# songweige/rich-text-to-image

Measured on AMD Instinct MI355X. Metric: denoising steps/sec (SDXL 1024^2, 50-step, 4 regions), higher is better.
Workload: dtype bf16; 1 GPU; SDXL RegionDiffusionXL 1024x1024, R=4 regions, inject_selfattn=0.5, 50-step Euler, CFG 5.0, 7 UNet forwards/step batched, random-init SDXL-base weights; global_batch=1, parallelism=seed-parallel x1 (1 weight broadcast, no per-step collectives), elide_dead_forwards=False

## Files before the change

### include/rtdiff.h

```cpp
#ifndef RTDIFF_H
#define RTDIFF_H
#include <stdint.h>
#ifdef __cplusplus
extern "C" {
#endif

#define RT_OK 0
#define RT_E_INVALID (-1)
#define RT_E_HIP (-2)
#define RT_E_STATE (-3)
#define RT_E_MISSING_WEIGHT (-4)
#define RT_E_UNSUPPORTED (-5)

#define RT_MAX_LEVELS 4
#define RT_MAX_STREAMS 16

enum { RT_DTYPE_F32 = 0, RT_DTYPE_F16 = 1, RT_DTYPE_BF16 = 2 };
enum { RT_SCHED_EULER = 0, RT_SCHED_PNDM = 1, RT_SCHED_DPMPP_1 = 2, RT_SCHED_DPMPP_2 = 3,
       RT_SCHED_EULER_A = 4, RT_SCHED_DPMPP_SDE_1 = 5, RT_SCHED_DPMPP_SDE_2 = 6 };

typedef struct rt_config {
    int n_levels;
    int block_out_channels[RT_MAX_LEVELS];
    int down_has_attn[RT_MAX_LEVELS];
// ... 108 lines not shown
int rt_trace_module_count(rt_engine* e);
int rt_trace_module_info(rt_engine* e, int idx, char* name, int name_cap, int* channels, int* downshift);

int rt_op_gemm(const void* A, const void* W, const float* bias, void* out, const void* res, const float* temb,
               int mode, int epi, int M, int N, int K, int lda, int ldw, int ldo, int ldres, int temb_ld,
               int rows_per_batch, int Hin, int Win, int Cin, int Hout, int Wout, void* stream);
int rt_op_attention(const void* Q, int ldq, const void* K, int ldk, const void* VT, int ldvt, void* O, int ldo,
                    const int* q_src_host, const int* k_src_host, const int* v_src_host, const int* wset_host,
                    const float* wabs, const float* wsgn, int B, int H, int N, int NK, int nk_valid, int DP, int cross,
                    void* stream);
int rt_op_attention_keys(const void* Q, int ldq, const void* K, int ldk, const void* VT, int ldvt, void* O, int ldo,
                         const int* q_src_host, const int* prompt_host, const int* wset_host, const float* wabs, const float* wsgn,
                         const int* key_counts_host, int B, int H, int N, int NK, int DP, void* stream);
int rt_op_ip_attention(const void* Q, int ldq, const void* Kip, int ldk, const void* VTip, int ldvt, void* O, int ldo,
                       const int* slot_host, const int* count_host, const float* scale_host, int B, int H, int N, int DP, void* stream);
int rt_op_identity_attention(const void* VT, int ldvt, void* O, int ldo, const int* entry_host, int n, int B, int H, int N, int DP, void* stream);
int rt_op_pag_fold(float* eps, int n_streams, int h, int w, const int* stream_host, const int* twin_host, const float* ratio_host, int n, void* stream);
int rt_op_lora_add(const void* X, int ldx, const void* down, int ldd, const void* up, int ldu, const float* alpha_over_rank,
                   const int* col_adapter, void* Y, int ldy, int form, const int* row_host, const float* scale_host, int B, int rows, int K,
                   int N, int R, int* launched, void* stream);
int rt_op_attention_units_plan(const int* q_src, const int* k_src, int B, int tokens, int DP, int mode, int* launch_of, int* unit_of, int* members_of);
int rt_op_gemm16_pick(int conv3x3, int epi, int streams, int rows_per_stream, int N, int K_or_Cin, int weights_on_rows, int* w_stationary);
int rt_op_split_plan(int conv3x3, int epi, int streams, int rows_per_stream, int N, int K_or_Cin, int* route, int* slices);
enum { RT_ROUTE_TILE = 0        ,
       RT_ROUTE_G16 = 1         ,
       RT_ROUTE_G16_UP2 = 2     ,
       RT_ROUTE_PATCH = 3       ,
       RT_ROUTE_PATCH_SPLIT = 4 ,
       RT_ROUTE_KSPLIT = 5      ,
       RT_ROUTE_TRIPLE = 6       };
int rt_op_gemm_route(int mode, int epi, int M, int N, int K, int lda, int ldw, int ldo, int rows_per_batch, int Hin, int Win, int Cin,
                     int Hout, int Wout, int* kind, int* variant_or_cfg, int* slices);
int rt_op_gemm16_variant(const void* A, const void* W, const float* bias, void* out, const void* res, int epi, int M, int N, int K, int lda,
                         int ldw, int ldo, int ldres, int weights_on_rows, int variant, int wstat, void* stream);
int rt_op_gemm_pair_pick(int streams_qk, int streams, int rows_per_stream, int Nqk, int Nv, int K);
int rt_op_gemm_qk_vt(const void* X, int ldx, int K, int rows_per_stream, const void* Wqk, const float* bqk, int Mqk, int Nqk, void* qk, int ldqk,
                     const void* Wv, int Nv, int M, void* vt, int ldvt, int* grouped, void* stream);
int rt_op_cross_attn_block(const void* x, const void* wq, const void* wo, const float* bo, const void* kcache, const void* vtcache, int ldvt,
                           const int* prompt_host, const int* wset_host, const float* wabs, const float* wsgn, const void* trunk_in_f16,
                           void* trunk_out_f16, void* q_scratch, void* o_scratch, int B, int N, int C, int H, int DP, void* stream);
int rt_op_groupnorm(const void* x1, const void* x2, int in_type, int C1, int C2, int G, int B, int HW,
                    const float* gamma, const float* beta, float eps, int silu, void* out_bf16, void* raw_out_bf16,
                    void* stream);
int rt_op_groupnorm_form(int in_type, int C1, int C2, int G, int B, int HW);

int rt_op_gemm_hilo(const void* A, const void* A_lo, const void* W, const void* W_lo, const float* bias, float* out_f32, void* pair_lo,
// ... 111 lines not shown
```

### rich-text-to-image_amd/csrc/common.h

```cpp
#pragma once
#include <hip/hip_runtime.h>
#include <stdint.h>
#include <stdio.h>
#include <string>
#include <stdexcept>

typedef uint16_t bf16_t;
typedef __attribute__((ext_vector_type(8))) __bf16 bf16x8;
typedef __attribute__((ext_vector_type(4))) __bf16 bf16x4;
typedef __attribute__((ext_vector_type(16))) float f32x16;
typedef __attribute__((ext_vector_type(4))) float f32x4;

#define RT_OK 0
#define RT_E_INVALID (-1)
#define RT_E_HIP (-2)
#define RT_E_STATE (-3)
#define RT_E_MISSING_WEIGHT (-4)
#define RT_E_UNSUPPORTED (-5)

struct rt_error : std::runtime_error {
    int code;
    rt_error(int c, const std::string& m) : std::runtime_error(m), code(c) {}
};

// ... 105 lines not shown
};
int gemm_ln_emit_bn(const GemmArgs& a);
bool gemm_ln_fold_ok(const GemmArgs& a);
bool gemm16_ln_variant_ok(const GemmArgs& a, int v);
void launch_ln_partials(const f16_t* x, bf16_t* xb, float* part, int rows, int C, int bn, hipStream_t st, int part_ld = 0);
void launch_ln_fold_derive(const bf16_t* W, int ldw, const float* bias, const float* gamma, const float* beta, int N, int K,
                           bf16_t* Wf, float* sc, hipStream_t st);
int gemm16_variant_bn(int v);
bool xattn_fused_supported(int C, int H, int DP, int tokens);
void launch_xattn_fused(const GemmArgs& a, hipStream_t st);
struct XBlockArgs {
    const bf16_t* x; const bf16_t* wq; const bf16_t* wo; const float* bo;
    const bf16_t* kc; const bf16_t* vt;
    const f16_t* res; f16_t* out;
    const float* wabs; const float* wsgn;
    int ldk, ldvt, ldres, ldo;
    int M, tokens, nk_valid, C, H;
    int prompt[RT_MAXB], wset[RT_MAXB];
};
bool xblock_supported(int C, int H, int DP, int tokens);
void launch_xblock(const XBlockArgs& a, hipStream_t st);
void launch_gemm(const GemmArgs& a, hipStream_t st);
struct GemmRoute {
    enum Kind { G16, PATCH, PATCH_SPLIT, KSPLIT, TILE, TRIPLE, G16_UP2 };
    Kind kind = TILE;
    int variant = -1, wstat = 0;
    int slices = 1;
    int cfg = -1;
};
GemmRoute gemm_route(const GemmArgs& a);
bool gemm_pair_output_ok(const GemmArgs& a);
size_t gemm_splitk_scratch_floats(const GemmArgs& a);
void gemm_force_config(int cfg);
enum DebugBit {
    DBG_CONV_IMPLICIT = 0,
    DBG_NO_GEMM16 = 1,
    DBG_NO_SPLIT = 2,
    DBG_CONV_NO_GEMM16 = 3,
    DBG_NO_XATTN_FUSED = 4,
    DBG_STORE_TWO_PASS = 5,
    DBG_STORE_ONE_PASS = 6,
    DBG_TRIPLE = 7,
    DBG_TRIPLE_GEMM16 = 8,
    DBG_TRIPLE_PATCH = 9,
    DBG_CONV3P_NO_TN4 = 10,
    DBG_GN_CHUNK_128 = 11,
    DBG_G16_NO_DEEP = 12,
    DBG_NO_PAIR = 13,
    DBG_ATTN_NO_PRIO = 14,
    DBG_TRIPLE_DENSE = 15,
    DBG_XBLOCK = 16,
    DBG_STORE_OWN_STATS = 17,
    DBG_STORE_APPLY_V1 = 18,
    DBG_NO_CROSS77 = 19,
    DBG_C77_ONE_TILE = 20,
    DBG_C77_TWO_HEADS = 21,
    DBG_NO_LNFOLD = 22,
    DBG_GN_TWO_LAUNCH = 23,
    DBG_ATTN_UNITS = 24,
    DBG_G16_TALL = 27,
    DBG_NO_CHUNK_SPLIT = 28,
    DBG_NO_CHUNK_HALVES = 29,
    DBG_SPLIT_NO_SMALL_ROWS = 30,
};
enum DebugBit2 {
    DBG2_NO_UP2_PHASE = 0,
};
static inline int debug_bit(int flags, int bit) { return (flags >> bit) & 1; }
void gemm_set_debug(int flags);
void gemm_set_debug2(int flags);
bool gemm_lnfold_enabled();
bool gemm_xblock_enabled();
bool gemm_xattn_enabled();
#define RT_G16_NVAR 14
bool gemm16_supported(const GemmArgs& a);
int gemm16_pick(const GemmArgs& a, int weights_on_rows, int* wstat);
void launch_gemm16_variant(const GemmArgs& a, int variant, int wstat, hipStream_t st);
int gemm16_pick_up2(const GemmArgs& a);
void launch_gemm16_up2(const GemmArgs& a, int variant, hipStream_t st);
int gemm16_pair_variant(const GemmArgs& a, int va, int wa, const GemmArgs& b, int vb, int wb);
void launch_gemm16_pair(const GemmArgs& a, const GemmArgs& b, int pair, hipStream_t st);
int gemm_pair_grouped(const GemmArgs& a, const GemmArgs& b);
void launch_gemm_pair(const GemmArgs& a, const GemmArgs& b, hipStream_t st);

struct AttnArgs {
    const bf16_t* Q;  int ldq;
    const bf16_t* K;  int ldk;
    const bf16_t* VT; int ldvt;
    bf16_t* O;        int ldo;
    int q_src[RT_MAXB], k_src[RT_MAXB], v_src[RT_MAXB], wset[RT_MAXB];
    unsigned char ng[RT_MAXB], gvs[RT_MAXB][4], gob[RT_MAXB][4];
    const float* wabs;
    const float* wsgn;
    int B, H, N;
    int NK;
    int nk_valid;
    int nkeys[RT_MAXB];
    int DP;
    int cross;
    int nqb;
    float* stats; int stats_b;
};
// ... 143 lines not shown
```

### rich-text-to-image_amd/csrc/engine.hip

```cpp
#include "common.h"
#include "../../include/rtdiff.h"
#include <map>
#include <mutex>
#include <vector>
#include <string>
#include <cmath>
#include <cstring>
#include <functional>
#include <algorithm>

static thread_local std::string g_create_error;
static thread_local std::string g_op_error;

struct Arena {
    char* base = nullptr;
    size_t off = 0, cap = 0;
    void* alloc(size_t bytes) {
        off = (off + 255) & ~(size_t)255;
        void* p = base ? base + off : (void*)(uintptr_t)(off + 256);
        off += bytes;
        if (base && off > cap) throw rt_error(RT_E_STATE, "arena overflow");
        return p;
    }
};
// ... 2112 lines not shown
                             int epi, int M, int N, int K, int lda, int ldw, int ldo, int ldres, int temb_ld, int rows_per_batch, int Hin,
                             int Win, int Cin, int Hout, int Wout) {
    GemmArgs g{}; g.A = (const bf16_t*)A; g.W = (const bf16_t*)W; g.bias = bias; g.out = out; g.res = res; g.temb = temb;
    g.zero = zero; g.mode = mode; g.epi = epi; g.M = M; g.N = N; g.K = K; g.lda = lda; g.ldw = ldw; g.ldo = ldo;
    g.ldres = ldres; g.temb_ld = temb_ld; g.rows_per_batch = rows_per_batch; g.Hin = Hin; g.Win = Win; g.Cin = Cin;
    g.Hout = Hout; g.Wout = Wout;
    return g;
}
int rt_op_gemm(const void* A, const void* W, const float* bias, void* out, const void* res, const float* temb, int mode,
               int epi, int M, int N, int K, int lda, int ldw, int ldo, int ldres, int temb_ld, int rows_per_batch, int Hin,
               int Win, int Cin, int Hout, int Wout, void* stream) {
    OP_TRY({
        const GemmArgs g = op_gemm_args(A, W, bias, out, res, temb, op_zero_page(), mode, epi, M, N, K, lda, ldw, ldo, ldres, temb_ld, rows_per_batch,
                                        Hin, Win, Cin, Hout, Wout);
        launch_gemm(g, (hipStream_t)stream);
    })
}
static int op_route_kind(const GemmRoute& r, int* v) {
    *v = -1;
    switch (r.kind) {
        case GemmRoute::TILE: *v = r.cfg; return RT_ROUTE_TILE;
        case GemmRoute::G16: *v = r.variant; return RT_ROUTE_G16;
        case GemmRoute::G16_UP2: *v = r.variant; return RT_ROUTE_G16_UP2;
        case GemmRoute::PATCH: return RT_ROUTE_PATCH;
        case GemmRoute::PATCH_SPLIT: return RT_ROUTE_PATCH_SPLIT;
        case GemmRoute::KSPLIT: return RT_ROUTE_KSPLIT;
        case GemmRoute::TRIPLE: return RT_ROUTE_TRIPLE;
    }
    return RT_ROUTE_TILE;
}
int rt_op_gemm_route(int mode, int epi, int M, int N, int K, int lda, int ldw, int ldo, int rows_per_batch, int Hin, int Win, int Cin, int Hout,
                     int Wout, int* kind, int* variant_or_cfg, int* slices) {
    try {
        if (mode < A_DENSE || mode > A_CONV3_S2P0 || epi < EPI_BF16 || epi > EPI_F16 || M <= 0 || N <= 0 || K <= 0) return RT_E_INVALID;
        if (mode != A_DENSE && (rows_per_batch <= 0 || Cin <= 0 || Hin <= 0 || Win <= 0 || Hout <= 0 || Wout <= 0)) return RT_E_INVALID;
        const GemmArgs g = op_gemm_args(nullptr, nullptr, nullptr, nullptr, nullptr, nullptr, nullptr, mode, epi, M, N, K, lda, ldw, ldo, 0, 0,
                                        rows_per_batch, Hin, Win, Cin, Hout, Wout);
        const GemmRoute r = gemm_route(g);
        int v = -1;
        const int k = op_route_kind(r, &v);
        if (kind) *kind = k;
        if (variant_or_cfg) *variant_or_cfg = v;
        if (slices) *slices = r.slices;
        return RT_OK;
    } catch (...) { return RT_E_INVALID; }
}
// ... 129 lines not shown
}
int rt_op_attention_keys(const void* Q, int ldq, const void* K, int ldk, const void* VT, int ldvt, void* O, int ldo, const int* q_src,
                         const int* prompt, const int* wset, const float* wabs, const float* wsgn, const int* key_counts, int B, int H,
                         int N, int NK, int DP, void* stream) {
    OP_TRY({
        RT_REQUIRE(B >= 1 && B <= RT_MAXB && key_counts, "rt_op_attention_keys: batch / key counts");
        RT_REQUIRE(NK == 96 || NK == 192 || NK == 288, "rt_op_attention_keys: NK must be 96, 192 or 288 rows per prompt");
        int p[RT_MAXB], ws[RT_MAXB];
        for (int b = 0; b < B; ++b) {
            RT_REQUIRE(op_key_count_ok(key_counts[b], NK), "rt_op_attention_keys: a key count must be 77 per 96-row chunk of NK");
            p[b] = prompt ? prompt[b] : b; ws[b] = wset ? wset[b] : -1;
        }
        RT_REQUIRE(!q_src, "rt_op_attention_keys: cross launches read Q of their own batch entry (q_src must be NULL)");
        launch_cross(unet_cross_attn_args(AttnIO{(const bf16_t*)Q, ldq, (const bf16_t*)K, ldk, (const bf16_t*)VT, ldvt, (bf16_t*)O, ldo}, p, ws, key_counts, wabs, wsgn,
                                          B, H, N, NK, DP),
                     cross_route(H * DP, H, DP, DP, N, NK, key_counts, B, false, false, false), (hipStream_t)stream);
    })
}
static bool query_args(GemmArgs& g, int mode, int epi, int streams, int rows_per_stream, int N, int K_or_Cin, int weights_on_rows) {
    const int M = streams * rows_per_stream;
    if (mode != A_DENSE) {
        int side = 1; while (side * side < rows_per_stream) ++side;
        if (side * side != rows_per_stream || (mode == A_CONV3_UP2 && side % 2)) return false;
        const int in = mode == A_CONV3_UP2 ? side / 2 : side;
        g = unet_conv3_args(nullptr, nullptr, mode, op_mat(nullptr, nullptr, N, 9 * K_or_Cin), streams, in, in, K_or_Cin, nullptr, epi);
        g.weights_on_rows = weights_on_rows;
    } else if (weights_on_rows) {
        g = unet_vt_args(nullptr, rows_per_stream, op_mat(nullptr, nullptr, N, K_or_Cin), nullptr, K_or_Cin, M, nullptr, M);
        g.epi = epi;
    } else g = unet_dense_args(nullptr, rows_per_stream, nullptr, K_or_Cin, op_mat(nullptr, nullptr, N, K_or_Cin), M, nullptr, N, epi);
    return true;
}
int rt_op_split_plan(int conv3x3, int epi, int streams, int rows_per_stream, int N, int K_or_Cin, int* route, int* slices) {
    try {
        GemmArgs g;
        if (!query_args(g, conv3x3 == 3 ? A_CONV3_UP2 : conv3x3 ? A_CONV3 : A_DENSE, epi, streams, rows_per_stream, N, K_or_Cin, 0)) return RT_E_INVALID;
        const GemmRoute r = gemm_route(g);
        const int kind = r.kind == GemmRoute::KSPLIT ? 1 : r.kind == GemmRoute::PATCH_SPLIT ? 2 : 0;
        if (route) *route = kind;
        if (slices) *slices = kind ? r.slices : 1;
        return RT_OK;
    } catch (...) { return RT_E_INVALID; }
}
int rt_op_gemm16_pick(int conv3x3, int epi, int streams, int rows_per_stream, int N, int K_or_Cin, int weights_on_rows, int* w_stationary) {
    try {
        GemmArgs g;
        if (!query_args(g, conv3x3 ? A_CONV3 : A_DENSE, epi, streams, rows_per_stream, N, K_or_Cin, weights_on_rows)) return -2;
        int ws = 0;
        const int v = gemm16_pick(g, weights_on_rows, &ws);
        if (w_stationary) *w_stationary = ws;
        return v;
    } catch (...) { return -3; }
}
int rt_op_gemm16_variant(const void* A, const void* W, const float* bias, void* out, const void* res, int epi, int M, int N, int K, int lda,
                         int ldw, int ldo, int ldres, int weights_on_rows, int variant, int wstat, void* stream) {
    OP_TRY({
        GemmArgs g = unet_dense_args(op_zero_page(), 0, (const bf16_t*)A, lda, op_mat(W, bias, N, K), M, out, ldo, epi, res, ldres);
        g.ldw = ldw; g.weights_on_rows = weights_on_rows;
        if (variant < 0) { int ws = 0; variant = gemm16_pick(g, weights_on_rows, &ws); wstat = ws; RT_REQUIRE(variant >= 0, "rt_op_gemm16_variant: the family has no tile for this shape"); }
        launch_gemm16_variant(g, variant, wstat, (hipStream_t)stream);
    })
}
int rt_op_gemm_pair_pick(int streams_qk, int streams, int rows_per_stream, int Nqk, int Nv, int K) {
// ... 282 lines not shown
```

### rich-text-to-image_amd/csrc/gemm.hip

```cpp
#include "common.h"
#include <algorithm>
#include <cmath>
#include <map>
#include <tuple>
#include <type_traits>



#define BK 64
#ifndef RT_ABLATE
#define RT_ABLATE 0
#endif

template <int EPI, int TM, int TN, int NWC, int LDS_BYTES, bool PATCH = false>
__device__ __forceinline__ void gemm_epilogue(const GemmArgs& p, f32x16 (&acc)[TM][TN], int wrow0, int wcol0, int lane, int wave_c,
                                              char* smem, int prow_base = 0, int pW = 0) {
    auto grow = [&](int r) { return PATCH ? prow_base + (r >> 4) * pW + (r & 15) : r; };
    constexpr bool F16 = EPI == EPI_F16;
    constexpr bool F32 = EPI == EPI_F32 || F16;
    constexpr int ES = F32 ? 4 : 2;
    constexpr int TO = EPI == EPI_GEGLU ? TN / 2 : TN;
    static_assert(EPI != EPI_GEGLU || TN % 2 == 0, "GEGLU needs value/gate tile pairs in one wave");
    constexpr int MAXROW = LDS_BYTES / NWC / 32;
    constexpr int TS_RAW = (MAXROW - 16) / (32 * ES);
// ... 1050 lines not shown
        case A_CONV3_S2P0 * 8 + EPI_F32: launch_me<A_CONV3_S2P0, EPI_F32>(a, cfg, st); break;
        default: throw rt_error(RT_E_UNSUPPORTED, "gemm: (operand mode, epilogue) combination not built");
    }
    HIP_CHECK(hipGetLastError());
}

static struct GemmSwitches {
    int force_cfg = -1;
    bool conv_patch = true;
    bool use16 = true;
    bool splitk = true;
    bool conv16 = true;
    bool xattn = true;
    bool triple = false, triple16 = false, triple_patch = false, triple_dense = false;
    bool pair = true;
    bool cross77 = true;
    bool xblock = false;
    bool split_small_rows = true;
    bool conv3p_tn4 = true;
    bool chunk_split = true;
    bool chunk_halves = true;
    bool lnfold = true;
    bool up2_phase = true;
} g_sw;
#ifdef RT_PROBE
int g_conv3p_tn = 0;
#endif
void gemm_set_debug(int flags) {
    auto on = [flags](int bit) { return debug_bit(flags, bit); };
    g_sw.conv_patch = !on(DBG_CONV_IMPLICIT); g_sw.use16 = !on(DBG_NO_GEMM16); g_sw.splitk = !on(DBG_NO_SPLIT); g_sw.conv16 = !on(DBG_CONV_NO_GEMM16);
    g_sw.xattn = !on(DBG_NO_XATTN_FUSED); g_sw.xblock = on(DBG_XBLOCK); g_sw.cross77 = !on(DBG_NO_CROSS77); g_sw.pair = !on(DBG_NO_PAIR);
    g_sw.triple = on(DBG_TRIPLE); g_sw.triple16 = on(DBG_TRIPLE_GEMM16); g_sw.triple_patch = on(DBG_TRIPLE_PATCH); g_sw.triple_dense = on(DBG_TRIPLE_DENSE);
    g_sw.split_small_rows = !on(DBG_SPLIT_NO_SMALL_ROWS); g_sw.conv3p_tn4 = !on(DBG_CONV3P_NO_TN4);
    g_sw.chunk_split = !on(DBG_NO_CHUNK_SPLIT); g_sw.chunk_halves = !on(DBG_NO_CHUNK_HALVES); g_sw.lnfold = !on(DBG_NO_LNFOLD);
}
void gemm_set_debug2(int flags) { g_sw.up2_phase = !debug_bit(flags, DBG2_NO_UP2_PHASE); }
void gemm_force_config(int cfg) { g_sw.force_cfg = cfg; }
bool gemm_cross77_enabled() { return g_sw.cross77; }
bool gemm_lnfold_enabled() { return g_sw.lnfold && g_sw.use16 && g_sw.force_cfg < 0; }
bool gemm_xblock_enabled() { return g_sw.xblock && g_sw.use16 && g_sw.force_cfg < 0; }
bool gemm_xattn_enabled() { return g_sw.xattn && g_sw.use16 && g_sw.force_cfg < 0; }

template <int EPI, bool UP2, int TN>
static void launch_conv3p_tn(const GemmArgs& a, int ntm, int slices, hipStream_t st) {
    constexpr int LDS = 2 * (UP2 ? 104 : 328) * 128 + 3 * 32 * TN * 128;
    static bool attr = false;
    if (!attr) {
        HIP_CHECK(hipFuncSetAttribute((const void*)conv3p_kernel<EPI, UP2, TN>, hipFuncAttributeMaxDynamicSharedMemorySize, LDS));
        attr = true;
    }
    hipLaunchKernelGGL((conv3p_kernel<EPI, UP2, TN>), dim3(ntm * cdiv(a.N, 32 * TN), slices), dim3(512), LDS, st, a);
}
template <int EPI, bool UP2>
static void launch_conv3p(const GemmArgs& a, hipStream_t st, int slices = 1) {
    const int ntm = (a.M / a.rows_per_batch) * (a.Hout / 16) * (a.Wout / 16) * slices;
    auto cost = [&](int tn_, double c) {
        const double r = (double)ntm * cdiv(a.N, 32 * tn_) / 256.0;
        if (r <= 1.0) return c;
        const double up = std::ceil(r);
// ... 109 lines not shown
    const int per = cdiv(nc1, 8);
    const int s = cdiv(nc1, per);
    return s >= 2 ? s : 0;
}

GemmRoute gemm_route(const GemmArgs& a) {
    const GemmSwitches& s = g_sw;
    const bool by_shape = s.force_cfg < 0, hilo = a.A_lo || a.W_lo;
    const int ksl = s.splitk ? splitk_slices(a) : 1;
    GemmRoute r{};
    if (hilo && (!by_shape || ksl > 1 || s.triple)) { r.kind = GemmRoute::TRIPLE; return r; }
    const bool conv16 = a.mode == A_CONV3 && ksl == 1 && by_shape && s.use16 && s.conv16 && s.conv_patch && !a.prefer_patch_conv &&
                        (r.variant = gemm16_pick(a, 0, &r.wstat)) >= 0;
    if (hilo) {
        bool fused;
        if (conv16) fused = !s.triple16;
        else if (a.mode == A_DENSE) fused = s.use16 && !s.triple_dense && gemm16_pick(a, a.weights_on_rows, &r.wstat) >= 0;
        else fused = conv_patch_eligible(a) && !s.triple_patch;
        if (!fused) { r.kind = GemmRoute::TRIPLE; return r; }
    }
    if (conv16) { r.kind = GemmRoute::G16; return r; }
    if (a.mode == A_CONV3_UP2 && a.W_up2 && !hilo && ksl == 1 && by_shape && s.use16 && s.conv16 && s.conv_patch && s.up2_phase && !a.prefer_patch_conv &&
        (r.variant = gemm16_pick_up2(a)) >= 0) { r.kind = GemmRoute::G16_UP2; return r; }
    const int chunks = by_shape ? conv3p_split_slices(a, ksl) : 0;
    if (chunks > 1) { r.kind = GemmRoute::PATCH_SPLIT; r.slices = chunks; return r; }
    if (conv_patch_eligible(a) && ksl == 1) { r.kind = GemmRoute::PATCH; return r; }
    if (ksl > 1) { r.kind = GemmRoute::KSPLIT; r.slices = ksl; return r; }
    if (by_shape && s.use16 && (r.variant = gemm16_pick(a, a.weights_on_rows, &r.wstat)) >= 0) { r.kind = GemmRoute::G16; return r; }
    r.kind = GemmRoute::TILE; r.cfg = pick_config(a);
    return r;
}

static GemmArgs single_pass(const GemmArgs& a) { GemmArgs b = a; b.A_lo = nullptr; b.W_lo = nullptr; return b; }
static size_t split_floats(const GemmArgs& a, const GemmRoute& r) {
    return r.kind == GemmRoute::PATCH_SPLIT || r.kind == GemmRoute::KSPLIT ? (size_t)r.slices * a.M * ((a.N + 3) & ~3) : 0;
}
size_t gemm_splitk_scratch_floats(const GemmArgs& a) {
    const GemmRoute r = gemm_route(a);
    return r.kind == GemmRoute::TRIPLE ? gemm_splitk_scratch_floats(single_pass(a)) : split_floats(a, r);
}
static bool pair_output_ok(const GemmArgs& a, const GemmRoute& r) { return r.kind == GemmRoute::PATCH && a.epi == EPI_F32 && g_sw.force_cfg < 0; }
bool gemm_pair_output_ok(const GemmArgs& a) { return pair_output_ok(a, gemm_route(a)); }
static int ln_variant(const GemmArgs& a, const GemmRoute& r) { return r.kind == GemmRoute::G16 && !a.A_lo && !a.W_lo && !a.pair_lo ? r.variant : -1; }
int gemm_ln_emit_bn(const GemmArgs& a_in) {
    GemmArgs a = a_in; a.ln_part = nullptr; a.ln_emit = (float*)(uintptr_t)256;
    const int v = ln_variant(a, gemm_route(a));
// ... 78 lines not shown
    RT_REQUIRE(a.epi >= EPI_BF16 && a.epi <= EPI_F16, "gemm: unknown epilogue");
    if (a.epi == EPI_GEGLU) RT_REQUIRE(a.N % 16 == 0 && a.ldo % 8 == 0, "gemm: GEGLU output needs N % 16 == 0");
    RT_REQUIRE(a.ldo % 4 == 0 && ((uintptr_t)a.out & 15) == 0, "gemm: output must be 16-B aligned with ldo % 4 == 0");
    if (a.res) RT_REQUIRE(a.ldres % 4 == 0 && ((uintptr_t)a.res & 15) == 0, "gemm: residual must be 16-B aligned");
    if (a.bias) RT_REQUIRE(((uintptr_t)a.bias & 15) == 0, "gemm: bias must be 16-B aligned");
    if (a.temb) RT_REQUIRE(a.temb_ld % 4 == 0 && ((uintptr_t)a.temb & 15) == 0, "gemm: temb must be 16-B aligned");
    if (a.A_lo || a.W_lo) RT_REQUIRE(a.A_lo && a.W_lo && a.epi == EPI_F32, "gemm: a hi / lo contraction needs both low parts and an fp32 output");
}

static void launch_routed(const GemmArgs& a, const GemmRoute& r, hipStream_t st) {
    if (a.ln_part || a.ln_emit) RT_REQUIRE(gemm16_ln_variant_ok(a, ln_variant(a, r)), "gemm: LayerNorm fold asked of a route without it (gemm_ln_fold_ok / gemm_ln_emit_bn)");
    if (a.pair_lo) RT_REQUIRE(pair_output_ok(a, r) && ((uintptr_t)a.pair_lo & 7) == 0, "gemm: pair output is only built into the patch convolution (gemm_pair_output_ok)");
    switch (r.kind) {
        case GemmRoute::TRIPLE: {
            GemmArgs b = single_pass(a);
            launch_gemm(b, st);
            b.bias = nullptr; b.res = a.out; b.ldres = a.ldo;
            b.A = a.A_lo; launch_gemm(b, st);
            b.A = a.A; b.W = a.W_lo; launch_gemm(b, st);
            return;
        }
        case GemmRoute::G16: launch_gemm16_variant(a, r.variant, r.wstat, st); return;
        case GemmRoute::G16_UP2: launch_gemm16_up2(a, r.variant, st); return;
        case GemmRoute::PATCH:
            if (a.mode == A_CONV3_UP2) { if (a.epi == EPI_F16) launch_conv3p<EPI_F16, true>(a, st); else launch_conv3p<EPI_F32, true>(a, st); }
            else switch (a.epi) {
                case EPI_BF16: launch_conv3p<EPI_BF16, false>(a, st); break;
                case EPI_F32: launch_conv3p<EPI_F32, false>(a, st); break;
                case EPI_F16: launch_conv3p<EPI_F16, false>(a, st); break;
                default: launch_conv3p<EPI_BF16_TEMB, false>(a, st); break;
            }
            return;
        case GemmRoute::PATCH_SPLIT:
        case GemmRoute::KSPLIT: launch_split(a, r, st); return;
        case GemmRoute::TILE: launch_with_cfg(a, r.cfg, st); return;
    }
}
void launch_gemm(const GemmArgs& a, hipStream_t st) {
    check_gemm_args(a);
    launch_routed(a, gemm_route(a), st);
}

static int pair_grouped(const GemmArgs& a, const GemmRoute& ra, const GemmArgs& b, const GemmRoute& rb) {
    return g_sw.pair && ra.kind == GemmRoute::G16 && rb.kind == GemmRoute::G16 ? gemm16_pair_variant(a, ra.variant, ra.wstat, b, rb.variant, rb.wstat) : -1;
}
int gemm_pair_grouped(const GemmArgs& a, const GemmArgs& b) { return pair_grouped(a, gemm_route(a), b, gemm_route(b)); }
// ... 9 lines not shown
```

### rich-text-to-image_amd/csrc/gemm16.hip

```cpp
#include "common.h"
#include <algorithm>
#include <type_traits>

#define BK16 64

typedef __attribute__((ext_vector_type(4))) float f32x4_t;

#ifdef RT_G16_TIMING
__device__ long long g_g16_times[8192 * 8];
#define G16_T(i) { if (tid == 0) g_g16_times[blockIdx.x * 8 + (i)] = __builtin_readcyclecounter(); }
#else
#define G16_T(i)
#endif
#ifndef RT_G16_ABLATE
#define RT_G16_ABLATE 0
#endif

#define RT_G16_OOB 0x7fff0000

template <bool UNUSED>
static __device__ __forceinline__ f32x4_t g16_mma(const bf16x8& b, const bf16x8& a, const f32x4_t& c) {
    return __builtin_amdgcn_mfma_f32_16x16x32_bf16(b, a, c, 0, 0, 0);
}
#define RT_LNF_NONE 0
// ... 225 lines not shown
    }
    __syncthreads();
    if ((mode & 6) == 0) asm volatile("buffer_inv sc1" ::: "memory");
    else if (mode & 4) asm volatile("buffer_inv sc0" ::: "memory");
    gemm16_tile<A_DENSE, EPI_BF16, 7, 5, 2, 2, 2, 3, RT_LNF_ROWS>(pb, 0, blockIdx.x);
    if (tid == 0) g_chain_times[blockIdx.x * 4 + 3] = __builtin_readcyclecounter();
}
void launch_gemm16_chain(const GemmArgs& a, const GemmArgs& b, unsigned target, int mode, hipStream_t st) {
    constexpr int LDS = 3 * (224 + 160) * 128 + RT_LN_TAB;
    static bool attr = false;
    if (!attr) { HIP_CHECK(hipFuncSetAttribute((const void*)gemm16_chain_kernel<0>, hipFuncAttributeMaxDynamicSharedMemorySize, LDS)); attr = true; }
    RT_REQUIRE(a.M == b.M && a.N == 1280 && b.N == 1280 && a.M % 224 == 0 && (a.M / 224) * 8 == 256, "chain probe: 7168 x 1280 projections (256 workgroups, all resident)");
    hipLaunchKernelGGL(gemm16_chain_kernel<0>, dim3(256), dim3(512), LDS, st, a, b, target, mode);
    HIP_CHECK(hipGetLastError());
}
void gemm16_chain_read_times(long long* dst) { HIP_CHECK(hipMemcpyFromSymbol(dst, HIP_SYMBOL(g_chain_times), sizeof(long long) * 256 * 4)); }
void gemm16_chain_reset() { unsigned z[64] = {}; HIP_CHECK(hipMemcpyToSymbol(HIP_SYMBOL(g_chain_flags), z, sizeof(z))); }
#endif

int g_g16_deep = 1;
int g_g16_tall = 0;
void gemm16_set_tall(int on) { g_g16_tall = on; }
void gemm16_set_deep(int on) { g_g16_deep = on; }
struct G16Var { int BM, BN, WK, S, geglu_ok; };
static const G16Var kVar[RT_G16_NVAR] = {
    {224, 160, 2, 3, 0},
    {128, 160, 2, 3, 0},
    {224, 256, 1, 2, 1},
    {256, 256, 1, 2, 1},
    {224, 320, 1, 2, 0},
    {256, 320, 1, 2, 0},
    {160, 224, 2, 3, 0},
    {160, 128, 2, 3, 0},
    {128, 256, 1, 3, 1},
    {64, 160, 2, 3, 0},
    {128, 320, 1, 2, 0},
    {64, 320, 1, 3, 0},
    {160, 64, 2, 3, 0},
    {128, 160, 1, 2, 0},
};

template <int MODE, int EPI, int TMW, int TNW, int WM, int WN, int WK, int S, int LNF = 0>
static void launch_v(const GemmArgs& a, int wstat, hipStream_t st) {
    constexpr int BM = WM * TMW * 16, BN = WN * TNW * 16;
    constexpr int LDS = S * (BM + BN) * 128 + ((LNF == RT_LNF_ROWS || LNF == RT_LNF_COLS) ? RT_LN_TAB : 0);
    static bool attr = false;
// ... 118 lines not shown
    K kern = gemm16_kernel<A_DENSE, EPI_XATTN, 4, 5, 2, 4, 1, 2>;
    static bool attr = false;
    if (!attr) { HIP_CHECK(hipFuncSetAttribute((const void*)kern, hipFuncAttributeMaxDynamicSharedMemorySize, XA_LDS)); attr = true; }
    hipLaunchKernelGGL(kern, dim3(cdiv(a.M, 128) * (a.N / 320)), dim3(512), XA_LDS, st, a, 0);
    HIP_CHECK(hipGetLastError());
}
#else
bool xattn_fused_supported(int, int, int, int) { return false; }
void launch_xattn_fused(const GemmArgs&, hipStream_t) { throw rt_error(RT_E_UNSUPPORTED, "EPI_XATTN is built with `make PROBES=1` only"); }
bool xblock_supported(int, int, int, int) { return false; }
void launch_xblock(const XBlockArgs&, hipStream_t) { throw rt_error(RT_E_UNSUPPORTED, "xblock_kernel is built with `make PROBES=1` only"); }
#endif

static bool conv16_geometry(const GemmArgs& a) {
    return a.mode == A_CONV3 && a.Hin == a.Hout && a.Win == a.Wout && a.Cin % BK16 == 0 && a.K == 9 * a.Cin && a.rows_per_batch == a.Hout * a.Wout &&
           a.M % a.rows_per_batch == 0 && (long)a.M * a.Cin * 2 < (long)RT_G16_OOB;
}
bool gemm16_supported(const GemmArgs& a) {
    if (a.mode == A_CONV3) {
        if (!conv16_geometry(a)) return false;
        if (!(a.epi == EPI_BF16 || a.epi == EPI_F32 || a.epi == EPI_F16 || a.epi == EPI_BF16_TEMB)) return false;
        return a.ldw % 8 == 0;
    }
    if (a.mode != A_DENSE || a.K % (2 * BK16) != 0 || a.K < 4 * BK16) return false;
    if ((a.A_lo || a.W_lo) && !(a.A_lo && a.W_lo && a.epi == EPI_F32)) return false;
    if (!(a.epi == EPI_BF16 || a.epi == EPI_F32 || a.epi == EPI_F16 || a.epi == EPI_GEGLU)) return false;
    if (a.lda % 8 || a.ldw % 8) return false;
    if ((long)a.M * a.lda * 2 >= 0x7fffffffL || (long)a.N * a.ldw * 2 >= 0x7fffffffL) return false;
    return true;
}

static bool up2_geometry(const GemmArgs& a) {
    return a.mode == A_CONV3_UP2 && a.W_up2 && a.Hout == 2 * a.Hin && a.Wout == 2 * a.Win && a.Cin % BK16 == 0 && a.K == 9 * a.Cin &&
           a.rows_per_batch == a.Hout * a.Wout && a.M % a.rows_per_batch == 0 && (long)(a.M / 4) * a.Cin * 2 < (long)RT_G16_OOB &&
           (long)a.N * 4 * a.Cin * 2 < 0x7fffffffL && a.epi == EPI_F16 && !a.res && !a.A_lo && !a.W_lo && !a.pair_lo && !a.ln_part && !a.ln_emit &&
           a.N % 8 == 0 && a.ldo % 8 == 0 && ((uintptr_t)a.W_up2 & 15) == 0;
}
int gemm16_pick_up2(const GemmArgs& a) {
    if (!up2_geometry(a)) return -1;
    const int rps = a.Hin * a.Win;
    if (rps < 256) return -1;
    if (a.N % 320 == 0 && (long)cdiv(rps, 224) * (a.N / 320) >= 32) return 4;
    if (a.N % 160 == 0) return (long)cdiv(rps, 224) * (a.N / 160) >= 30 ? 0 : -1;
    return -1;
}
void launch_gemm16_up2(const GemmArgs& a, int v, hipStream_t st) {
    RT_REQUIRE(up2_geometry(a) && (v == 0 || v == 4), "gemm16: phase form of the 2x-upsample convolution (phase pack, fp16 output, no residual, Cin % 64 == 0; 224 x 160 / 224 x 320 tiles)");
    GemmArgs g = a;
    g.M = a.M / 4; g.rows_per_batch = a.Hin * a.Win; g.K = 4 * a.Cin; g.W = a.W_up2; g.ldw = 4 * a.Cin;
    if (v == 0) launch_v<A_CONV3_UP2, EPI_F16, 7, 5, 2, 2, 2, 3>(g, 0, st);
    else launch_v<A_CONV3_UP2, EPI_F16, 7, 5, 2, 4, 1, 2>(g, 0, st);
}

void launch_gemm16_variant(const GemmArgs& a, int v, int wstat, hipStream_t st) {
    RT_REQUIRE(gemm16_supported(a), "gemm16: problem outside the family's domain (dense K % 128 == 0, K >= 256; or a 3x3 stride-1 convolution with Cin % 64 == 0)");
    RT_REQUIRE(v >= 0 && v < RT_G16_NVAR, "gemm16: variant");
    RT_REQUIRE(!(a.ln_part && a.ln_emit), "gemm16: a launch consumes OR produces LayerNorm partials");
    if (a.ln_part) { launch_ln(a, v, wstat, a.weights_on_rows ? RT_LNF_COLS : RT_LNF_ROWS, st); return; }
    if (a.ln_emit) { launch_ln(a, v, wstat, RT_LNF_EMIT, st); return; }
    if (a.mode == A_CONV3) {
        RT_REQUIRE(kVar[v].WK == 1 || (a.K / BK16) % 2 == 0, "gemm16: the K-split class needs an even number of K tiles");
        switch (a.epi) {
            case EPI_BF16: launch_e<A_CONV3, EPI_BF16>(a, v, wstat, st); break;
            case EPI_F32: launch_e<A_CONV3, EPI_F32>(a, v, wstat, st); break;
            case EPI_F16: launch_e<A_CONV3, EPI_F16>(a, v, wstat, st); break;
            default: launch_e<A_CONV3, EPI_BF16_TEMB>(a, v, wstat, st); break;
        }
        return;
    }
    switch (a.epi) {
        case EPI_BF16: launch_e<A_DENSE, EPI_BF16>(a, v, wstat, st); break;
        case EPI_F32: launch_e<A_DENSE, EPI_F32>(a, v, wstat, st); break;
        case EPI_F16: launch_e<A_DENSE, EPI_F16>(a, v, wstat, st); break;
        default: launch_e<A_DENSE, EPI_GEGLU>(a, v, wstat, st); break;
    }
}

template <int TMW_A, int TNW_A, int S_A, int TMW_B, int TNW_B, bool LN = false>
static void launch_dual_v(const GemmArgs& a, const GemmArgs& b, hipStream_t st) {
    constexpr int BMA = 2 * TMW_A * 16, BNA = 4 * TNW_A * 16, BMB = 2 * TMW_B * 16, BNB = 2 * TNW_B * 16;
    constexpr int LDS_A = S_A * (BMA + BNA) * 128, LDS_B = 3 * (BMB + BNB) * 128, LDS = (LDS_A > LDS_B ? LDS_A : LDS_B) + (LN ? RT_LN_TAB : 0);
    static bool attr = false;
// ... 45 lines not shown
    const double nk = a.K / 64.0;
    auto cost = [&](int BMv, int BNv, double eff) {
        const long tiles = (long)cdiv(a.M, BMv) * cdiv(a.N, BNv);
        return (double)((tiles + 255) / 256) * (nk * (BMv + BNv) / 384.0 * eff + 12.0);
    };
    if (a.mode == A_CONV3) {
        const bool wide = a.N % 320 == 0 && (long)cdiv(rps, 224) * (a.N / 320) >= 32;
        if (wide) return 4;
        if (a.N % 160 == 0 && (a.K / BK16) % 2 == 0) return (long)cdiv(rps, 224) * (a.N / 160) >= 30 ? 0 : -1;
        if (a.N % 256 == 0) return (long)cdiv(rps, 224) * (a.N / 256) >= 30 ? 2 : -1;
        return -1;
    }
    if (weights_on_rows) {
        if (a.epi != EPI_BF16 || a.M % 160 != 0) return -1;
        if ((long)(a.M / 160) * cdiv(a.N, 64) <= 256) return 12;
        return cost(160, 224, 1.0) <= cost(160, 128, 1.2) ? 6 : 7;
    }
    if (a.epi == EPI_GEGLU) {
        if (a.N % 256 != 0) return -1;
        *wstat = (a.N / 256) % 8 == 0 ? 1 : (g_g16_tall ? 2 : 0);
        const double c2 = cost(224, 256, 1.0), c3 = cost(256, 256, 1.0), c8 = cost(128, 256, 1.2);
        return c2 <= c3 && c2 <= c8 ? 2 : (c3 <= c8 ? 3 : 8);
    }
    const bool wide320 = a.N % 320 == 0 && (long)cdiv(rps, 224) * (a.N / 320) >= 32;
    if (wide320) {
        static const int cand[4][3] = {{224, 320, 4}, {224, 256, 2}, {256, 256, 3}, {128, 256, 8}};
        int best = -1; double bc = 1e300;
        for (auto& c : cand) {
            if (a.N % c[1] != 0) continue;
            if (a.ln_emit && c[1] != 320) continue;
            const double cc = cost(c[0], c[1], c[0] == 128 ? 1.2 : 1.0);
            if (cc < bc) { bc = cc; best = c[2]; }
        }
        if (best >= 0 && (long)cdiv(a.M, kVar[best].BM) * (a.N / kVar[best].BN) <= 128) {
            if ((long)cdiv(a.M, 64) * (a.N / 320) <= 256) return 11;
            if ((long)cdiv(a.M, 128) * (a.N / 320) <= 256) return 10;
        }
        return best;
    }
    if (a.N % 160 == 0) {
        if ((long)cdiv(a.M, 64) * (a.N / 160) <= 256) return 9;
        return cost(224, 160, 1.0) <= cost(128, 160, 1.2) ? 0 : 1;
    }
    if (a.N % 256 == 0) {
        const double c2 = cost(224, 256, 1.0), c3 = cost(256, 256, 1.0), c8 = cost(128, 256, 1.2);
        return c2 <= c3 && c2 <= c8 ? 2 : (c3 <= c8 ? 3 : 8);
    }
    return -1;
}


#ifdef RT_G16_TIMING
void gemm16_read_times(long long* dst, int n) { HIP_CHECK(hipMemcpyFromSymbol(dst, HIP_SYMBOL(g_g16_times), (size_t)n * 8)); }
void gemm16_read_xa_segments(long long* dst, int n) { HIP_CHECK(hipMemcpyFromSymbol(dst, HIP_SYMBOL(g_xa_seg), (size_t)n * 8)); }
#endif
```

### rich-text-to-image_amd/engine.py

```python
import ctypes as C
import os

_HERE = os.path.dirname(os.path.abspath(__file__))
_LIB_PATH = os.path.join(_HERE, "librtdiff.so")
_lib = None

RT_MAX_LEVELS = 4
RT_MAX_STREAMS = 16
DTYPE_F32, DTYPE_F16, DTYPE_BF16 = 0, 1, 2
SCHED_EULER, SCHED_PNDM = 0, 1
PRED_EPSILON, PRED_V = 0, 1
PREDICTION_TYPES = {"epsilon": PRED_EPSILON, "v_prediction": PRED_V}
A_DENSE, A_CONV3, A_CONV3_S2, A_CONV3_UP2, A_CONV3_S2P0 = 0, 1, 2, 3, 4
EPI_BF16, EPI_F32, EPI_BF16_TEMB, EPI_GEGLU, EPI_F16 = 0, 1, 2, 3, 4

SD15_CONFIG = dict(
    in_channels=4, out_channels=4, block_out_channels=(320, 640, 1280, 1280),
    down_block_types=("CrossAttnDownBlock2D", "CrossAttnDownBlock2D", "CrossAttnDownBlock2D", "DownBlock2D"),
    up_block_types=("UpBlock2D", "CrossAttnUpBlock2D", "CrossAttnUpBlock2D", "CrossAttnUpBlock2D"),
    layers_per_block=2, transformer_layers_per_block=1, attention_head_dim=8, cross_attention_dim=768,
    norm_num_groups=32, norm_eps=1e-5, use_linear_projection=False, addition_embed_type=None,
    addition_time_embed_dim=None, projection_class_embeddings_input_dim=None)
SDXL_CONFIG = dict(
    in_channels=4, out_channels=4, block_out_channels=(320, 640, 1280),
# ... 38 lines not shown
        self.code = code


_SYMBOLS = [
    "rt_create", "rt_destroy", "rt_last_error", "rt_set_stream", "rt_synchronize", "rt_weight_count",
    "rt_weight_info", "rt_bind_weight", "rt_weights_missing", "rt_arena_info", "rt_arena_mark_bound",
    "rt_set_prompts", "rt_set_masks", "rt_set_fontsize", "rt_set_schedule", "rt_set_latents", "rt_get_latents",
    "rt_region_step", "rt_plain_step", "rt_unet_forward", "rt_op_gemm", "rt_op_attention", "rt_op_groupnorm",
    "rt_op_layernorm", "rt_op_layernorm_f16", "rt_op_small_linear", "rt_op_timestep_embed", "rt_op_last_error", "rt_profile_enable",
    "rt_profile_read", "rt_op_gemm_force_config", "rt_op_gemm_debug", "rt_attn_store_enable", "rt_attn_store_reset",
    "rt_attn_store_read", "rt_attn_module_count", "rt_attn_module_info", "rt_get_state_ptrs", "rt_background_blend", "rt_vae_create", "rt_vae_destroy",
    "rt_vae_last_error", "rt_vae_weight_count", "rt_vae_weight_info", "rt_vae_bind_weight", "rt_vae_synchronize", "rt_vae_decode",
    "rt_vae_color_guidance", "rt_vae_arena_info", "rt_vae_arena_mark_bound", "rt_op_cast_bf16", "rt_op_attention_probs_avg", "rt_op_embed", "rt_op_activation", "rt_op_causal_attention",
    "rt_op_cross_attn_block", "rt_op_gemm16_variant", "rt_op_gemm16_pick", "rt_op_split_plan", "rt_profile_read2", "rt_op_gemm_qk_vt", "rt_op_gemm_pair_pick",
    "rt_region_step_part", "rt_region_step_finish", "rt_eps_info", "rt_op_split_range",
    "rt_op_ln_gemm", "rt_op_gemm_emit_partials", "rt_op_ln_partials", "rt_op_probes_built", "rt_op_attention_units_plan",
    "rt_plain_step_part", "rt_plain_step_finish", "rt_vae_encoder_create", "rt_vae_encode", "rt_vae_posterior_sample",
    "rt_set_source", "rt_noise_latents", "rt_source_blend",
    "rt_op_gemm_debug2", "rt_op_pack_upconv", "rt_op_upconv",
    "rt_set_prompts_keys", "rt_op_attention_keys",
    "rt_set_noise_seed", "rt_op_step_noise",
    "rt_set_prediction", "rt_op_guided_prediction",
    "rt_op_attention_store_handover",
    "rt_op_gemm_route", "rt_op_groupnorm_form", "rt_op_cross_route",
    "rt_set_freeu", "rt_op_freeu",
    "rt_op_gemm_hilo", "rt_op_gemm_hilo_route", "rt_op_split_bf16", "rt_op_vae_groupnorm_nchunk", "rt_op_vae_groupnorm", "rt_op_vae_groupnorm_bwd",
    "rt_op_softmax_rows", "rt_op_softmax_bwd", "rt_op_transpose_bf16", "rt_op_sumpool2x2", "rt_op_pq_conv_fwd", "rt_op_pq_conv_bwd_update",
    "rt_op_color_loss_grad",
    "rt_set_image_prompts", "rt_op_ip_attention",
    "rt_unet_forward_trace", "rt_trace_module_count", "rt_trace_module_info",
    "rt_op_patchify", "rt_op_vit_embed", "rt_op_bidir_attention",
    "rt_op_latent_attention",
    "rt_set_control_hint", "rt_control_embedding_read", "rt_set_control_scales", "rt_op_control_add",
    "rt_op_lora_add", "rt_set_lora_columns", "rt_set_lora_scales", "rt_attn_cache_info",
    "rt_set_pag_layers", "rt_set_pag_scales", "rt_plain_streams", "rt_unet_forward_perturbed", "rt_op_identity_attention", "rt_op_pag_fold",
]


def load_library(path=None):
    global _lib
    if _lib is not None and path is None:
        return _lib
    p = path or os.environ.get("RTDIFF_LIB_PATH") or _LIB_PATH
    if not os.path.exists(p):
        raise RtError(-3, f"{p} not found: build it with `python __graft_entry__.py build` "
                          "(hipcc --offload-arch=gfx950); there is no fallback path")
    lib = C.CDLL(p)
# ... 847 lines not shown
```

Before: 22.19 steps/s.

## Route stride-2 3x3 convs and odd-K dense GEMMs to gemm16 matrix-core kernels

Adds a G16_S2 route that runs the stride-2 3x3 downsample convolutions through the gemm16 matrix-core kernel family with 224x160 or 128x160 tiles, when the geometry and tile count allow it. It also relaxes gemm16 eligibility for dense GEMMs whose K is an odd multiple of the K tile, restricted to single-K-warp variants, so those shapes stop falling back to the generic tile path. A planning query API and debug switches are added. The new routes bring more template instantiations and tile-choice heuristics that may not beat the old path on every shape.

```diff
diff --git a/include/rtdiff.h b/include/rtdiff.h
--- a/include/rtdiff.h
+++ b/include/rtdiff.h
@@ -154,6 +154,8 @@
 int rt_op_attention_units_plan(const int* q_src, const int* k_src, int B, int tokens, int DP, int mode, int* launch_of, int* unit_of, int* members_of);
 int rt_op_gemm16_pick(int conv3x3, int epi, int streams, int rows_per_stream, int N, int K_or_Cin, int weights_on_rows, int* w_stationary);
 int rt_op_split_plan(int conv3x3, int epi, int streams, int rows_per_stream, int N, int K_or_Cin, int* route, int* slices);
+int rt_op_plan_route(int conv3x3, int epi, int streams, int rows_per_stream, int N, int K_or_Cin, int* kind, int* variant_or_cfg, int* slices,
+                     long long* scratch_floats);
 enum { RT_ROUTE_TILE = 0        ,
        RT_ROUTE_G16 = 1         ,
        RT_ROUTE_G16_UP2 = 2     ,
diff --git a/rich-text-to-image_amd/csrc/common.h b/rich-text-to-image_amd/csrc/common.h
--- a/rich-text-to-image_amd/csrc/common.h
+++ b/rich-text-to-image_amd/csrc/common.h
@@ -151,7 +151,7 @@
 void launch_xblock(const XBlockArgs& a, hipStream_t st);
 void launch_gemm(const GemmArgs& a, hipStream_t st);
 struct GemmRoute {
-    enum Kind { G16, PATCH, PATCH_SPLIT, KSPLIT, TILE, TRIPLE, G16_UP2 };
+    enum Kind { G16, PATCH, PATCH_SPLIT, KSPLIT, TILE, TRIPLE, G16_UP2, G16_S2 };
     Kind kind = TILE;
     int variant = -1, wstat = 0;
     int slices = 1;
@@ -194,6 +194,9 @@
 };
 enum DebugBit2 {
     DBG2_NO_UP2_PHASE = 0,
+    DBG2_NO_S2_GEMM16 = 1,
+    DBG2_NO_ODDK_GEMM16 = 2,
+    DBG2_G16_ANY_SHAPE = 3,
 };
 static inline int debug_bit(int flags, int bit) { return (flags >> bit) & 1; }
 void gemm_set_debug(int flags);
@@ -207,6 +210,10 @@
 void launch_gemm16_variant(const GemmArgs& a, int variant, int wstat, hipStream_t st);
 int gemm16_pick_up2(const GemmArgs& a);
 void launch_gemm16_up2(const GemmArgs& a, int variant, hipStream_t st);
+int gemm16_pick_s2(const GemmArgs& a);
+void launch_gemm16_s2(const GemmArgs& a, int variant, hipStream_t st);
+void gemm16_set_oddk(int on);
+void gemm16_set_any_shape(int on);
 int gemm16_pair_variant(const GemmArgs& a, int va, int wa, const GemmArgs& b, int vb, int wb);
 void launch_gemm16_pair(const GemmArgs& a, const GemmArgs& b, int pair, hipStream_t st);
 int gemm_pair_grouped(const GemmArgs& a, const GemmArgs& b);
diff --git a/rich-text-to-image_amd/csrc/engine.hip b/rich-text-to-image_amd/csrc/engine.hip
--- a/rich-text-to-image_amd/csrc/engine.hip
+++ b/rich-text-to-image_amd/csrc/engine.hip
@@ -2158,6 +2158,7 @@
         case GemmRoute::TILE: *v = r.cfg; return RT_ROUTE_TILE;
         case GemmRoute::G16: *v = r.variant; return RT_ROUTE_G16;
         case GemmRoute::G16_UP2: *v = r.variant; return RT_ROUTE_G16_UP2;
+        case GemmRoute::G16_S2: *v = r.variant; return RT_ROUTE_G16;
         case GemmRoute::PATCH: return RT_ROUTE_PATCH;
         case GemmRoute::PATCH_SPLIT: return RT_ROUTE_PATCH_SPLIT;
         case GemmRoute::KSPLIT: return RT_ROUTE_KSPLIT;
@@ -2333,7 +2334,7 @@
     if (mode != A_DENSE) {
         int side = 1; while (side * side < rows_per_stream) ++side;
         if (side * side != rows_per_stream || (mode == A_CONV3_UP2 && side % 2)) return false;
-        const int in = mode == A_CONV3_UP2 ? side / 2 : side;
+        const int in = mode == A_CONV3_UP2 ? side / 2 : mode == A_CONV3_S2 ? side * 2 : side;
         g = unet_conv3_args(nullptr, nullptr, mode, op_mat(nullptr, nullptr, N, 9 * K_or_Cin), streams, in, in, K_or_Cin, nullptr, epi);
         g.weights_on_rows = weights_on_rows;
     } else if (weights_on_rows) {
@@ -2345,11 +2346,26 @@
 int rt_op_split_plan(int conv3x3, int epi, int streams, int rows_per_stream, int N, int K_or_Cin, int* route, int* slices) {
     try {
         GemmArgs g;
-        if (!query_args(g, conv3x3 == 3 ? A_CONV3_UP2 : conv3x3 ? A_CONV3 : A_DENSE, epi, streams, rows_per_stream, N, K_or_Cin, 0)) return RT_E_INVALID;
+        if (!query_args(g, conv3x3 == 3 ? A_CONV3_UP2 : conv3x3 == 2 ? A_CONV3_S2 : conv3x3 ? A_CONV3 : A_DENSE, epi, streams, rows_per_stream, N, K_or_Cin, 0)) return RT_E_INVALID;
         const GemmRoute r = gemm_route(g);
         const int kind = r.kind == GemmRoute::KSPLIT ? 1 : r.kind == GemmRoute::PATCH_SPLIT ? 2 : 0;
         if (route) *route = kind;
         if (slices) *slices = kind ? r.slices : 1;
+        return RT_OK;
+    } catch (...) { return RT_E_INVALID; }
+}
+int rt_op_plan_route(int conv3x3, int epi, int streams, int rows_per_stream, int N, int K_or_Cin, int* kind, int* variant_or_cfg, int* slices,
+                     long long* scratch_floats) {
+    try {
+        GemmArgs g;
+        if (conv3x3 < 0 || conv3x3 > 3 || !query_args(g, conv3x3 == 3 ? A_CONV3_UP2 : conv3x3 == 2 ? A_CONV3_S2 : conv3x3 ? A_CONV3 : A_DENSE, epi, streams, rows_per_stream, N, K_or_Cin, 0)) return RT_E_INVALID;
+        const GemmRoute r = gemm_route(g);
+        int v = -1;
+        const int k = op_route_kind(r, &v);
+        if (kind) *kind = k;
+        if (variant_or_cfg) *variant_or_cfg = v;
+        if (slices) *slices = r.slices;
+        if (scratch_floats) *scratch_floats = (long long)gemm_splitk_scratch_floats(g);
         return RT_OK;
     } catch (...) { return RT_E_INVALID; }
 }
diff --git a/rich-text-to-image_amd/csrc/gemm.hip b/rich-text-to-image_amd/csrc/gemm.hip
--- a/rich-text-to-image_amd/csrc/gemm.hip
+++ b/rich-text-to-image_amd/csrc/gemm.hip
@@ -1096,6 +1096,8 @@
     bool chunk_halves = true;
     bool lnfold = true;
     bool up2_phase = true;
+    bool s2_g16 = true;
+    bool g16_any = false;
 } g_sw;
 #ifdef RT_PROBE
 int g_conv3p_tn = 0;
@@ -1108,7 +1110,10 @@
     g_sw.split_small_rows = !on(DBG_SPLIT_NO_SMALL_ROWS); g_sw.conv3p_tn4 = !on(DBG_CONV3P_NO_TN4);
     g_sw.chunk_split = !on(DBG_NO_CHUNK_SPLIT); g_sw.chunk_halves = !on(DBG_NO_CHUNK_HALVES); g_sw.lnfold = !on(DBG_NO_LNFOLD);
 }
-void gemm_set_debug2(int flags) { g_sw.up2_phase = !debug_bit(flags, DBG2_NO_UP2_PHASE); }
+void gemm_set_debug2(int flags) {
+    g_sw.up2_phase = !debug_bit(flags, DBG2_NO_UP2_PHASE); g_sw.s2_g16 = !debug_bit(flags, DBG2_NO_S2_GEMM16); g_sw.g16_any = debug_bit(flags, DBG2_G16_ANY_SHAPE);
+    gemm16_set_oddk(!debug_bit(flags, DBG2_NO_ODDK_GEMM16)); gemm16_set_any_shape(g_sw.g16_any);
+}
 void gemm_force_config(int cfg) { g_sw.force_cfg = cfg; }
 bool gemm_cross77_enabled() { return g_sw.cross77; }
 bool gemm_lnfold_enabled() { return g_sw.lnfold && g_sw.use16 && g_sw.force_cfg < 0; }
@@ -1264,6 +1269,10 @@
     if (conv16) { r.kind = GemmRoute::G16; return r; }
     if (a.mode == A_CONV3_UP2 && a.W_up2 && !hilo && ksl == 1 && by_shape && s.use16 && s.conv16 && s.conv_patch && s.up2_phase && !a.prefer_patch_conv &&
         (r.variant = gemm16_pick_up2(a)) >= 0) { r.kind = GemmRoute::G16_UP2; return r; }
+    if (a.mode == A_CONV3_S2 && !hilo && (ksl == 1 || s.g16_any) && by_shape && s.use16 && s.conv16 && s.s2_g16 &&
+        (r.variant = gemm16_pick_s2(a)) >= 0) { r.kind = GemmRoute::G16_S2; return r; }
+    if (s.g16_any && a.mode == A_DENSE && a.K % 128 != 0 && !hilo && ksl > 1 && by_shape && s.use16 &&
+        (r.variant = gemm16_pick(a, a.weights_on_rows, &r.wstat)) >= 0) { r.kind = GemmRoute::G16; return r; }
     const int chunks = by_shape ? conv3p_split_slices(a, ksl) : 0;
     if (chunks > 1) { r.kind = GemmRoute::PATCH_SPLIT; r.slices = chunks; return r; }
     if (conv_patch_eligible(a) && ksl == 1) { r.kind = GemmRoute::PATCH; return r; }
@@ -1388,6 +1397,7 @@
         }
         case GemmRoute::G16: launch_gemm16_variant(a, r.variant, r.wstat, st); return;
         case GemmRoute::G16_UP2: launch_gemm16_up2(a, r.variant, st); return;
+        case GemmRoute::G16_S2: launch_gemm16_s2(a, r.variant, st); return;
         case GemmRoute::PATCH:
             if (a.mode == A_CONV3_UP2) { if (a.epi == EPI_F16) launch_conv3p<EPI_F16, true>(a, st); else launch_conv3p<EPI_F32, true>(a, st); }
             else switch (a.epi) {
diff --git a/rich-text-to-image_amd/csrc/gemm16.hip b/rich-text-to-image_amd/csrc/gemm16.hip
--- a/rich-text-to-image_amd/csrc/gemm16.hip
+++ b/rich-text-to-image_amd/csrc/gemm16.hip
@@ -271,6 +271,10 @@
 int g_g16_tall = 0;
 void gemm16_set_tall(int on) { g_g16_tall = on; }
 void gemm16_set_deep(int on) { g_g16_deep = on; }
+int g_g16_oddk = 1;
+int g_g16_any = 0;
+void gemm16_set_oddk(int on) { g_g16_oddk = on; }
+void gemm16_set_any_shape(int on) { g_g16_any = on; }
 struct G16Var { int BM, BN, WK, S, geglu_ok; };
 static const G16Var kVar[RT_G16_NVAR] = {
     {224, 160, 2, 3, 0},
@@ -435,7 +439,8 @@
         if (!(a.epi == EPI_BF16 || a.epi == EPI_F32 || a.epi == EPI_F16 || a.epi == EPI_BF16_TEMB)) return false;
         return a.ldw % 8 == 0;
     }
-    if (a.mode != A_DENSE || a.K % (2 * BK16) != 0 || a.K < 4 * BK16) return false;
+    if (a.mode != A_DENSE || a.K % BK16 != 0 || a.K < 4 * BK16) return false;
+    if (a.K % (2 * BK16) != 0 && !(g_g16_oddk && !a.A_lo && !a.W_lo && !a.ln_part && !a.ln_emit && !a.weights_on_rows && a.epi != EPI_GEGLU)) return false;
     if ((a.A_lo || a.W_lo) && !(a.A_lo && a.W_lo && a.epi == EPI_F32)) return false;
     if (!(a.epi == EPI_BF16 || a.epi == EPI_F32 || a.epi == EPI_F16 || a.epi == EPI_GEGLU)) return false;
     if (a.lda % 8 || a.ldw % 8) return false;
@@ -465,12 +470,35 @@
     else launch_v<A_CONV3_UP2, EPI_F16, 7, 5, 2, 4, 1, 2>(g, 0, st);
 }
 
+static bool s2_geometry(const GemmArgs& a) {
+    return a.mode == A_CONV3_S2 && a.Hin % 2 == 0 && a.Win % 2 == 0 && a.Hout == a.Hin / 2 && a.Wout == a.Win / 2 && a.Cin % BK16 == 0 && a.Cin >= BK16 &&
+           a.K == 9 * a.Cin && a.rows_per_batch == a.Hout * a.Wout && a.M % a.rows_per_batch == 0 &&
+           (long)(a.M / a.rows_per_batch) * a.Hin * a.Win * a.Cin * 2 < (long)RT_G16_OOB && (long)a.N * a.ldw * 2 < 0x7fffffffL && a.ldw % 8 == 0 &&
+           (a.epi == EPI_F16 || a.epi == EPI_BF16) && !a.A_lo && !a.W_lo && !a.pair_lo && !a.ln_part && !a.ln_emit && a.N % 160 == 0 && a.ldo % 8 == 0 &&
+           !a.res;
+}
+int gemm16_pick_s2(const GemmArgs& a) {
+    if (!s2_geometry(a)) return -1;
+    if (g_g16_any) return 0;
+    const int rps = a.rows_per_batch;
+    if (rps < 256) return -1;
+    if ((long)cdiv(rps, 224) * (a.N / 160) >= 30) return 0;
+    if ((long)cdiv(rps, 128) * (a.N / 160) >= 30) return 1;
+    return -1;
+}
+void launch_gemm16_s2(const GemmArgs& a, int v, hipStream_t st) {
+    RT_REQUIRE(s2_geometry(a) && (v == 0 || v == 1), "gemm16: stride-2 3x3 convolution (even map, Cin % 64 == 0, N % 160 == 0, fp16 / bf16 output; 224 x 160 / 128 x 160 tiles)");
+    if (a.epi == EPI_F16) { if (v == 0) launch_v<A_CONV3_S2, EPI_F16, 7, 5, 2, 2, 2, 3>(a, 0, st); else launch_v<A_CONV3_S2, EPI_F16, 4, 5, 2, 2, 2, 3>(a, 0, st); }
+    else { if (v == 0) launch_v<A_CONV3_S2, EPI_BF16, 7, 5, 2, 2, 2, 3>(a, 0, st); else launch_v<A_CONV3_S2, EPI_BF16, 4, 5, 2, 2, 2, 3>(a, 0, st); }
+}
+
 void launch_gemm16_variant(const GemmArgs& a, int v, int wstat, hipStream_t st) {
     RT_REQUIRE(gemm16_supported(a), "gemm16: problem outside the family's domain (dense K % 128 == 0, K >= 256; or a 3x3 stride-1 convolution with Cin % 64 == 0)");
     RT_REQUIRE(v >= 0 && v < RT_G16_NVAR, "gemm16: variant");
     RT_REQUIRE(!(a.ln_part && a.ln_emit), "gemm16: a launch consumes OR produces LayerNorm partials");
     if (a.ln_part) { launch_ln(a, v, wstat, a.weights_on_rows ? RT_LNF_COLS : RT_LNF_ROWS, st); return; }
     if (a.ln_emit) { launch_ln(a, v, wstat, RT_LNF_EMIT, st); return; }
+    if (a.mode == A_DENSE) RT_REQUIRE(kVar[v].WK == 1 || a.K % (2 * BK16) == 0, "gemm16: the K-split class needs an even number of K tiles");
     if (a.mode == A_CONV3) {
         RT_REQUIRE(kVar[v].WK == 1 || (a.K / BK16) % 2 == 0, "gemm16: the K-split class needs an even number of K tiles");
         switch (a.epi) {
@@ -562,7 +590,8 @@
         const double c2 = cost(224, 256, 1.0), c3 = cost(256, 256, 1.0), c8 = cost(128, 256, 1.2);
         return c2 <= c3 && c2 <= c8 ? 2 : (c3 <= c8 ? 3 : 8);
     }
-    const bool wide320 = a.N % 320 == 0 && (long)cdiv(rps, 224) * (a.N / 320) >= 32;
+    const bool oddk = a.K % (2 * BK16) != 0;
+    const bool wide320 = a.N % 320 == 0 && ((long)cdiv(rps, 224) * (a.N / 320) >= 32 || (oddk && g_g16_any));
     if (wide320) {
         static const int cand[4][3] = {{224, 320, 4}, {224, 256, 2}, {256, 256, 3}, {128, 256, 8}};
         int best = -1; double bc = 1e300;
@@ -578,6 +607,7 @@
         }
         return best;
     }
+    if (oddk) return -1;
     if (a.N % 160 == 0) {
         if ((long)cdiv(a.M, 64) * (a.N / 160) <= 256) return 9;
         return cost(224, 160, 1.0) <= cost(128, 160, 1.2) ? 0 : 1;
diff --git a/rich-text-to-image_amd/engine.py b/rich-text-to-image_amd/engine.py
--- a/rich-text-to-image_amd/engine.py
+++ b/rich-text-to-image_amd/engine.py
@@ -84,7 +84,7 @@
     "rt_set_noise_seed", "rt_op_step_noise",
     "rt_set_prediction", "rt_op_guided_prediction",
     "rt_op_attention_store_handover",
-    "rt_op_gemm_route", "rt_op_groupnorm_form", "rt_op_cross_route",
+    "rt_op_gemm_route", "rt_op_groupnorm_form", "rt_op_cross_route", "rt_op_plan_route",
     "rt_set_freeu", "rt_op_freeu",
     "rt_op_gemm_hilo", "rt_op_gemm_hilo_route", "rt_op_split_bf16", "rt_op_vae_groupnorm_nchunk", "rt_op_vae_groupnorm", "rt_op_vae_groupnorm_bwd",
     "rt_op_softmax_rows", "rt_op_softmax_bwd", "rt_op_transpose_bf16", "rt_op_sumpool2x2", "rt_op_pq_conv_fwd", "rt_op_pq_conv_bwd_update",
```

Measured after the change: 22.27 steps/s (median of 6 runs). Within noise of the previous version (+0.3%).
